# tudelft-iv/CCVPE

Measured on NVIDIA B200. Metric: VIGOR pairs/sec (CVM_VIGOR forward + pose decode, 320x640 panorama + 512x512 aerial), higher is better.
Workload: dtype bf16

## Files before the change

ccvpe_b200/csrc/encoder_ops.cu:

```cuda
#include <cstdlib>
#include <cstring>

#include "common.cuh"

namespace ccvpe {

constexpr float kSeFixedScale = 1048576.f;
__device__ __forceinline__ unsigned long long se_fixed(float v) {
  return (unsigned long long)__float2ll_rn(v * kSeFixedScale);
}

__global__ void __launch_bounds__(256)
bias_silu_nhwc_kernel(const __nv_bfloat16* __restrict__ x, const __nv_bfloat16* __restrict__ bias,
                      __nv_bfloat16* __restrict__ y, int64_t y_sb, int64_t y_sh, int64_t y_sw, int H, int W, int C,
                      int pix_per_block, long long* __restrict__ chan_sum) {
  extern __shared__ unsigned long long s_sum[];
  const int G = C >> 3;
  const int lanes = blockDim.x / G;
  const int cg = threadIdx.x % G, pl = threadIdx.x / G;
  const int b = blockIdx.y;
  const int HW = H * W;
  const int p_lo = blockIdx.x * pix_per_block;
  const int p_hi = min(HW, p_lo + pix_per_block);
  if (chan_sum) {
    for (int c = threadIdx.x; c < C; c += blockDim.x) s_sum[c] = 0ull;
    __syncthreads();
  }
  float bv[8] = {0.f, 0.f, 0.f, 0.f, 0.f, 0.f, 0.f, 0.f};
  if (bias && pl < lanes) {
    uint4 q = *reinterpret_cast<const uint4*>(bias + cg * 8);
    const __nv_bfloat162* h = reinterpret_cast<const __nv_bfloat162*>(&q);
#pragma unroll
    for (int j = 0; j < 4; ++j) {
      float2 f = __bfloat1622float2(h[j]);
      bv[2 * j] = f.x;
      bv[2 * j + 1] = f.y;
    }
  }
  float acc[8] = {0.f, 0.f, 0.f, 0.f, 0.f, 0.f, 0.f, 0.f};
  if (pl < lanes) {
    const __nv_bfloat16* xb = x + (int64_t)b * HW * C + cg * 8;
    __nv_bfloat16* yb = y + (int64_t)b * y_sb + cg * 8;
    constexpr int U = 4;
    for (int p0 = p_lo + pl; p0 < p_hi; p0 += lanes * U) {
      uint4 q[U];
#pragma unroll
      for (int u = 0; u < U; ++u) {
        const int p = p0 + u * lanes;
        if (p < p_hi) q[u] = __ldcs(reinterpret_cast<const uint4*>(xb + (int64_t)p * C));
      }
#pragma unroll
      for (int u = 0; u < U; ++u) {
        const int p = p0 + u * lanes;
        if (p >= p_hi) break;
        __nv_bfloat162* h = reinterpret_cast<__nv_bfloat162*>(&q[u]);
#pragma unroll
        for (int j = 0; j < 4; ++j) {
          float2 f = __bfloat1622float2(h[j]);
          float a0 = f.x + bv[2 * j], a1 = f.y + bv[2 * j + 1];
          a0 = __fdividef(a0, 1.f + __expf(-a0));
          a1 = __fdividef(a1, 1.f + __expf(-a1));
          h[j] = __floats2bfloat162_rn(a0, a1);
          if (chan_sum) {
            float2 r = __bfloat1622float2(h[j]);
            acc[2 * j] += r.x;
            acc[2 * j + 1] += r.y;
          }
        }
        const int hh = p / W, ww = p - hh * W;
        *reinterpret_cast<uint4*>(yb + hh * y_sh + ww * y_sw) = q[u];
      }
    }
  }
  if (chan_sum) {
    if (pl < lanes) {
#pragma unroll
      for (int j = 0; j < 8; ++j) atomicAdd(&s_sum[cg * 8 + j], se_fixed(acc[j]));
    }
    __syncthreads();
    for (int c = threadIdx.x; c < C; c += blockDim.x)
      atomicAdd(reinterpret_cast<unsigned long long*>(chan_sum) + (int64_t)b * C + c, s_sum[c]);
  }
}

}

extern "C" int ccvpe_bias_silu_nhwc(const void* x, const void* bias, void* y, int64_t y_sb, int64_t y_sh, int64_t y_sw,
                                    int B, int H, int W, int C, int64_t* chan_sum, void* stream) {
  using namespace ccvpe;
  CCVPE_REQUIRE(x && y, "ccvpe_bias_silu_nhwc: null pointer");
  CCVPE_REQUIRE(B > 0 && H > 0 && W > 0 && C > 0 && C % 8 == 0 && C <= 2048, "ccvpe_bias_silu_nhwc: bad shape B=%d H=%d W=%d C=%d",
                B, H, W, C);
  CCVPE_REQUIRE(aligned16(x) && aligned16(y) && aligned16(bias), "ccvpe_bias_silu_nhwc: pointers must be 16-byte aligned");
  CCVPE_REQUIRE(y_sw % 8 == 0 && y_sh % 8 == 0 && y_sb % 8 == 0, "ccvpe_bias_silu_nhwc: output strides must be multiples of 8");
  const int G = C / 8;
  CCVPE_REQUIRE(G <= 256, "ccvpe_bias_silu_nhwc: C too large");
  const int lanes = 256 / G;
  const int64_t HW = (int64_t)H * W;
  int blocks_x = (int)((8LL * sm_count() + B - 1) / B);
  int64_t ppb = (HW + blocks_x - 1) / blocks_x;
  ppb = (ppb + lanes - 1) / lanes * lanes;
  if (ppb < lanes) ppb = lanes;
  blocks_x = (int)((HW + ppb - 1) / ppb);
  bias_silu_nhwc_kernel<<<dim3(blocks_x, B), 256, chan_sum ? C * sizeof(unsigned long long) : 0, (cudaStream_t)stream>>>(
      (const __nv_bfloat16*)x, (const __nv_bfloat16*)bias, (__nv_bfloat16*)y, y_sb, y_sh, y_sw, H, W, C, (int)ppb, reinterpret_cast<long long*>(chan_sum));
  CCVPE_LAUNCH_CHECK("bias_silu_nhwc_kernel");
  return CCVPE_OK;
}

namespace ccvpe {

__device__ __forceinline__ float dw_tanh(float x) {
  float y;
  asm("tanh.approx.f32 %0, %1;" : "=f"(y) : "f"(x));
  return y;
}

template <int V> struct DwVec;
template <> struct DwVec<8> { using type = uint4; };
template <> struct DwVec<4> { using type = uint2; };
template <int V>
__device__ __forceinline__ void dw_widen(const typename DwVec<V>::type& q, uint64_t (&f)[V / 2]);
template <>
__device__ __forceinline__ void dw_widen<8>(const uint4& q, uint64_t (&f)[4]) {
  f[0] = bf16x2_to_f32x2(q.x);
  f[1] = bf16x2_to_f32x2(q.y);
  f[2] = bf16x2_to_f32x2(q.z);
  f[3] = bf16x2_to_f32x2(q.w);
}
template <>
__device__ __forceinline__ void dw_widen<4>(const uint2& q, uint64_t (&f)[2]) {
  f[0] = bf16x2_to_f32x2(q.x);
  f[1] = bf16x2_to_f32x2(q.y);
}

template <int K, int S, int V>
__global__ void __launch_bounds__(256, V == 8 ? 2 : 3)
dwconv_bias_silu_kernel(const __nv_bfloat16* __restrict__ x, int64_t x_sb, int64_t x_sh, int64_t x_sw,
                        const __nv_bfloat16* __restrict__ w, const __nv_bfloat16* __restrict__ bias,
                        __nv_bfloat16* __restrict__ y, int Ho, int Wo, int C, int CG, int strips_per_block,
                        long long* __restrict__ chan_sum) {
  using vec_t = typename DwVec<V>::type;
  constexpr int P = V / 2;
  constexpr int TW = 4;
  constexpr int IW = (TW - 1) * S + K;
  extern __shared__ __align__(16) float s_part[];
  const int CC = CG * V;
  float* s_w = s_part + (blockDim.x / CG) * CC;
  const int G = C / V;
  const int g0 = blockIdx.z * CG;
  const int gn = min(CG, G - g0);
  const int lanes = blockDim.x / CG;
  const int cl = threadIdx.x % CG, pl = threadIdx.x / CG;
  const int cg = g0 + cl;
  const bool active = pl < lanes && cl < gn;
  const int b = blockIdx.y;
  {
    const int q4 = gn * V / 4, n_items = K * K * q4;
#pragma unroll 1
    for (int i0 = threadIdx.x; i0 < n_items; i0 += 4 * blockDim.x) {
      uint2 v[4];
      int dst[4];
#pragma unroll
      for (int u = 0; u < 4; ++u) {
        const int i = i0 + u * blockDim.x;
        const int ii = i < n_items ? i : 0;
        const int tap = ii / q4, c4 = ii - tap * q4;
        v[u] = __ldg(reinterpret_cast<const uint2*>(w + (int64_t)tap * C + g0 * V) + c4);
        dst[u] = i < n_items ? tap * CC + c4 * 4 : -1;
      }
#pragma unroll
      for (int u = 0; u < 4; ++u)
        if (dst[u] >= 0)
          *reinterpret_cast<float4*>(s_w + dst[u]) =
              make_float4(0.5f * __uint_as_float(v[u].x << 16), 0.5f * __uint_as_float(v[u].x & 0xffff0000u),
                          0.5f * __uint_as_float(v[u].y << 16), 0.5f * __uint_as_float(v[u].y & 0xffff0000u));
    }
  }
  const int strips_row = (Wo + TW - 1) / TW;
  const int n_strips = Ho * strips_row;
  const int s_lo = blockIdx.x * strips_per_block;
  const int s_hi = min(n_strips, s_lo + strips_per_block);
  __syncthreads();
  float csum[V];
#pragma unroll
  for (int j = 0; j < V; ++j) csum[j] = 0.f;
  if (active) {
    uint64_t bv[P];
    dw_widen<V>(*reinterpret_cast<const vec_t*>(bias + cg * V), bv);
#pragma unroll
    for (int j = 0; j < P; ++j) {
      float lo, hi;
      unpack_f32x2(bv[j], lo, hi);
      bv[j] = pack_f32x2(0.5f * lo, 0.5f * hi);
    }
    const __nv_bfloat16* xb = x + (int64_t)b * x_sb + cg * V;
    __nv_bfloat16* yb = y + (int64_t)b * Ho * Wo * C + cg * V;
    const float* wt = s_w + cl * V;
    const int iw_max = (Wo - 1) * S + K - 1;
    const int sw = (int)x_sw;
    for (int sidx = s_lo + pl; sidx < s_hi; sidx += lanes) {
      const int ho = sidx / strips_row;
      const int wo0 = (sidx - ho * strips_row) * TW;
      uint64_t acc[TW][P];
#pragma unroll
      for (int t = 0; t < TW; ++t)
#pragma unroll
        for (int j = 0; j < P; ++j) acc[t][j] = bv[j];
      const int ix_max = iw_max - wo0 * S;
      const __nv_bfloat16* xrow = xb + (int64_t)(ho * S) * x_sh + (int64_t)(wo0 * S) * x_sw;
#pragma unroll 1
      for (int ky = 0; ky < K; ++ky, xrow += x_sh) {
        vec_t xin[IW];
#pragma unroll
        for (int ix = 0; ix < IW; ++ix)
          xin[ix] = __ldg(reinterpret_cast<const vec_t*>(xrow + min(ix, ix_max) * sw));
        uint64_t xf[IW][P];
#pragma unroll
        for (int kx = 0; kx < K; ++kx) {
          uint64_t wv[P];
// ... 177 lines not shown
            if (ky >= 0 && ky < K) {
              const uint2 wq = dwt_lds64(sw + (uint32_t)(ky * K + kx) * 128u);
              const uint64_t w0 = bf16x2_to_f32x2(wq.x), w1 = bf16x2_to_f32x2(wq.y);
#pragma unroll
              for (int t = 0; t < TW; ++t) {
                acc[r][t][0] = ffma2(xf[t + kx][0], w0, acc[r][t][0]);
                acc[r][t][1] = ffma2(xf[t + kx][1], w1, acc[r][t][1]);
              }
            }
          }
        }
      }
      const int ho0 = th_i * p.oth + ph * TH, wo0 = tw_i * p.otw + pw * TW;
#pragma unroll
      for (int r = 0; r < TH; ++r) {
        const int ho = ho0 + r;
        if (ho < p.Ho) {
          __nv_bfloat16* yrow = p.y + (((int64_t)b * p.Ho + ho) * p.Wo) * p.C + c0 + cg * 4;
#pragma unroll
          for (int t = 0; t < TW; ++t) {
            const int wo = wo0 + t;
            if (wo < p.Wo) {
              uint2 q;
              __nv_bfloat162* h = reinterpret_cast<__nv_bfloat162*>(&q);
#pragma unroll
              for (int j = 0; j < 2; ++j) {
                float a0, a1;
                unpack_f32x2(acc[r][t][j], a0, a1);
                a0 *= 0.5f;
                a1 *= 0.5f;
                a0 = fmaf(a0, dw_tanh(a0), a0);
                a1 = fmaf(a1, dw_tanh(a1), a1);
                h[j] = __floats2bfloat162_rn(a0, a1);
                const float2 rr = __bfloat1622float2(h[j]);
                csum[2 * j] += rr.x;
                csum[2 * j + 1] += rr.y;
              }
              *reinterpret_cast<uint2*>(yrow + (int64_t)wo * p.C) = q;
            }
          }
        }
      }
    }
    if (p.chan_sum) {
#pragma unroll
      for (int j = 0; j < 4; ++j) s_part[pt * DWT_CB + cg * 4 + j] = csum[j];
    }
    __syncthreads();
    if (p.chan_sum && tid < DWT_CB && c0 + tid < p.C) {
      float tot = 0.f;
#pragma unroll
      for (int l = 0; l < DWT_PT; ++l) tot += s_part[l * DWT_CB + tid];
      atomicAdd(reinterpret_cast<unsigned long long*>(p.chan_sum) + (int64_t)b * p.C + c0 + tid, se_fixed(tot));
    }
  }
}

static bool dwt_plan(int K, int Ho, int Wo, int C, int B, DwTileParams* p) {
  double best = 1e30;
  bool found = false;
  for (int ptw = 1; ptw <= DWT_PT; ++ptw) {
    const int pth = DWT_PT / ptw;
    const int otw = ptw * DWT_TW, oth = pth * DWT_TH;
    const int itw = otw + K - 1, ith = oth + K - 1;
    const int stage = (K * K + ith * itw) * 128;
    if (stage > DWT_STAGE_LIMIT) continue;
    const int tiles_w = (Wo + otw - 1) / otw, tiles_h = (Ho + oth - 1) / oth;
    const double cost = (double)tiles_w * tiles_h * (ith * itw + 2.0 * DWT_PT * DWT_TW * DWT_TH);
    if (cost < best) {
      best = cost;
      found = true;
      p->ptw = ptw; p->pth = pth; p->otw = otw; p->oth = oth; p->itw = itw; p->ith = ith;
      p->tiles_w = tiles_w; p->tiles_h = tiles_h; p->stage_bytes = stage;
    }
  }
  if (!found) return false;
  p->cblocks = (C + DWT_CB - 1) / DWT_CB;
  const int64_t total = (int64_t)p->tiles_w * p->tiles_h * p->cblocks * B;
  if (total > (1LL << 30)) return false;
  p->total_items = (int)total;
  return true;
}

__global__ void __launch_bounds__(512)
se_gate_scale_kernel(const long long* __restrict__ chan_sum, float inv_hw, const __nv_bfloat16* __restrict__ w_red,
                     const __nv_bfloat16* __restrict__ b_red, const __nv_bfloat16* __restrict__ w_se_t,
                     const __nv_bfloat16* __restrict__ b_se, const __nv_bfloat16* __restrict__ w_proj,
                     __nv_bfloat16* __restrict__ wg, int mid, int R, int cout, int rows_per_block) {
  extern __shared__ __align__(16) float s_se[];
  float* s_mean = s_se;
  float* s_h = s_se + mid;
  const int b = blockIdx.x, tid = threadIdx.x, lane = tid & 31, warp = tid >> 5;
  for (int m = tid; m < mid; m += blockDim.x) s_mean[m] = __ll2float_rn(chan_sum[(int64_t)b * mid + m]) * (inv_hw * (1.f / kSeFixedScale));
  __syncthreads();
  const int n_warps = blockDim.x >> 5;
  for (int r = warp; r < R; r += n_warps) {
    const __nv_bfloat16* wr = w_red + (int64_t)r * mid;
    float acc = 0.f;
    for (int m0 = lane * 8; m0 < mid; m0 += 256) {
      const uint4 q = __ldg(reinterpret_cast<const uint4*>(wr + m0));
      const __nv_bfloat162* hq = reinterpret_cast<const __nv_bfloat162*>(&q);
#pragma unroll
      for (int j = 0; j < 4; ++j) {
        const float2 f = __bfloat1622float2(hq[j]);
        acc = fmaf(f.x, s_mean[m0 + 2 * j], acc);
        acc = fmaf(f.y, s_mean[m0 + 2 * j + 1], acc);
      }
    }
#pragma unroll
    for (int o = 16; o > 0; o >>= 1) acc += __shfl_xor_sync(0xffffffffu, acc, o);
    if (lane == 0) {
      const float v = acc + __bfloat162float(b_red[r]);
      s_h[r] = __fdividef(v, 1.f + __expf(-v));
    }
  }
  __syncthreads();
  for (int m = tid; m < mid; m += blockDim.x) {
    float acc = __bfloat162float(b_se[m]);
#pragma unroll 8
    for (int r = 0; r < R; ++r) acc = fmaf(__bfloat162float(__ldg(w_se_t + (int64_t)r * mid + m)), s_h[r], acc);
    s_mean[m] = __fdividef(1.f, 1.f + __expf(-acc));
  }
  __syncthreads();
  const int c_lo = blockIdx.y * rows_per_block, c_hi = min(cout, c_lo + rows_per_block);
  const int vec_per_row = mid >> 3;
  const int total = (c_hi - c_lo) * vec_per_row;
  const uint4* src = reinterpret_cast<const uint4*>(w_proj + (int64_t)c_lo * mid);
  uint4* dst = reinterpret_cast<uint4*>(wg + ((int64_t)b * cout + c_lo) * mid);
  for (int i = tid; i < total; i += blockDim.x) {
    const int m0 = (i % vec_per_row) * 8;
    uint4 q = __ldg(src + i);
    __nv_bfloat162* hq = reinterpret_cast<__nv_bfloat162*>(&q);
#pragma unroll
    for (int j = 0; j < 4; ++j) {
      const float2 f = __bfloat1622float2(hq[j]);
      hq[j] = __floats2bfloat162_rn(f.x * s_mean[m0 + 2 * j], f.y * s_mean[m0 + 2 * j + 1]);
    }
    dst[i] = q;
  }
}

__global__ void __launch_bounds__(1024)
se_gate_kernel(const long long* __restrict__ chan_sum, float inv_hw, const __nv_bfloat16* __restrict__ w_red,
               const __nv_bfloat16* __restrict__ b_red, const __nv_bfloat16* __restrict__ w_se_t,
               const __nv_bfloat16* __restrict__ b_se, float* __restrict__ gate, int mid, int R) {
  extern __shared__ __align__(16) float s_se[];
  float* s_mean = s_se;
  float* s_h = s_se + mid;
  const int b = blockIdx.x, tid = threadIdx.x, lane = tid & 31, warp = tid >> 5;
  for (int m = tid; m < mid; m += blockDim.x) s_mean[m] = __ll2float_rn(chan_sum[(int64_t)b * mid + m]) * (inv_hw * (1.f / kSeFixedScale));
  __syncthreads();
  const int n_warps = blockDim.x >> 5;
  for (int r = warp; r < R; r += n_warps) {
    const __nv_bfloat16* wr = w_red + (int64_t)r * mid;
    float acc = 0.f;
    for (int m0 = lane * 8; m0 < mid; m0 += 256) {
      const uint4 q = __ldg(reinterpret_cast<const uint4*>(wr + m0));
      const __nv_bfloat162* hq = reinterpret_cast<const __nv_bfloat162*>(&q);
#pragma unroll
      for (int j = 0; j < 4; ++j) {
        const float2 f = __bfloat1622float2(hq[j]);
        acc = fmaf(f.x, s_mean[m0 + 2 * j], acc);
        acc = fmaf(f.y, s_mean[m0 + 2 * j + 1], acc);
      }
    }
#pragma unroll
// ... 115 lines not shown

extern "C" int ccvpe_stem_conv_silu_nhwc(const float* x, int B, int H, int W, const float* w, const float* bias, int CO,
                                         void* out, int in_pad_lo, int in_pad_hi, int out_pad_lo, int out_pad_hi,
                                         int circular, void* stream) {
  using namespace ccvpe;
  CCVPE_REQUIRE(x && w && bias && out, "ccvpe_stem_conv_silu_nhwc: null pointer");
  CCVPE_REQUIRE(B > 0 && H >= 3 && W >= 3 && B <= 65535, "ccvpe_stem_conv_silu_nhwc: bad shape B=%d H=%d W=%d", B, H, W);
  CCVPE_REQUIRE(CO == 32, "ccvpe_stem_conv_silu_nhwc: CO=%d unsupported (EfficientNet-B0 stem has 32 channels)", CO);
  CCVPE_REQUIRE(in_pad_lo >= 0 && in_pad_lo <= 2 && in_pad_hi >= 0 && in_pad_hi <= 2 && out_pad_lo >= 0 && out_pad_hi >= 0,
                "ccvpe_stem_conv_silu_nhwc: bad padding");
  CCVPE_REQUIRE(aligned16(out), "ccvpe_stem_conv_silu_nhwc: out must be 16-byte aligned");
  const int Ho = (H + in_pad_lo + in_pad_hi - 3) / 2 + 1, Wo = (W + in_pad_lo + in_pad_hi - 3) / 2 + 1;
  CCVPE_REQUIRE(!circular || (out_pad_lo <= Wo && out_pad_hi <= Wo), "ccvpe_stem_conv_silu_nhwc: wrap wider than the image");
  const int Hp = Ho + out_pad_lo + out_pad_hi, Wp = Wo + out_pad_lo + out_pad_hi;
  cudaStream_t st = (cudaStream_t)stream;
  StemTcParams tp;
  memset(&tp, 0, sizeof(tp));
  tp.x = x; tp.w = w; tp.bias = bias; tp.out = (__nv_bfloat16*)out;
  tp.B = B; tp.H = H; tp.W = W; tp.Ho = Ho; tp.Wo = Wo; tp.in_lo = in_pad_lo; tp.out_lo = out_pad_lo; tp.Hp = Hp; tp.Wp = Wp;
  return stem_tcgen05(tp, circular != 0, false, st);
}

extern "C" int ccvpe_stem_conv_silu_u8_nhwc(const uint8_t* x, int B, int H, int Wsrc, int crop_w, const int32_t* shift,
                                            const float* mean_host, const float* std_host, const float* w, const float* bias,
                                            int CO, void* out, int in_pad_lo, int in_pad_hi, int out_pad_lo, int out_pad_hi,
                                            int circular, void* stream) {
  using namespace ccvpe;
  CCVPE_REQUIRE(x && w && bias && out && mean_host && std_host, "ccvpe_stem_conv_silu_u8_nhwc: null pointer");
  const int W = crop_w;
  CCVPE_REQUIRE(B > 0 && H >= 3 && W >= 3 && W <= Wsrc && B <= 65535, "ccvpe_stem_conv_silu_u8_nhwc: bad shape B=%d H=%d W=%d Wsrc=%d",
                B, H, W, Wsrc);
  CCVPE_REQUIRE(CO == 32, "ccvpe_stem_conv_silu_u8_nhwc: CO=%d unsupported (EfficientNet-B0 stem has 32 channels)", CO);
  CCVPE_REQUIRE(in_pad_lo >= 0 && in_pad_lo <= 2 && in_pad_hi >= 0 && in_pad_hi <= 2 && out_pad_lo >= 0 && out_pad_hi >= 0,
                "ccvpe_stem_conv_silu_u8_nhwc: bad padding");
  CCVPE_REQUIRE(aligned16(out), "ccvpe_stem_conv_silu_u8_nhwc: out must be 16-byte aligned");
  const int Ho = (H + in_pad_lo + in_pad_hi - 3) / 2 + 1, Wo = (W + in_pad_lo + in_pad_hi - 3) / 2 + 1;
  CCVPE_REQUIRE(!circular || (out_pad_lo <= Wo && out_pad_hi <= Wo), "ccvpe_stem_conv_silu_u8_nhwc: wrap wider than the image");
  const int Hp = Ho + out_pad_lo + out_pad_hi, Wp = Wo + out_pad_lo + out_pad_hi;
  StemTcParams tp;
  memset(&tp, 0, sizeof(tp));
  tp.x8 = x; tp.shift = shift; tp.Wsrc = Wsrc;
  for (int c = 0; c < 3; ++c) {
    tp.sc[c] = 1.f / (255.f * std_host[c]);
    tp.sh[c] = -mean_host[c] / std_host[c];
  }
  tp.w = w; tp.bias = bias; tp.out = (__nv_bfloat16*)out;
  tp.B = B; tp.H = H; tp.W = W; tp.Ho = Ho; tp.Wo = Wo; tp.in_lo = in_pad_lo; tp.out_lo = out_pad_lo; tp.Hp = Hp; tp.Wp = Wp;
  return stem_tcgen05(tp, circular != 0, true, (cudaStream_t)stream);
}

extern "C" int ccvpe_pointwise_silu_nhwc(const void* x, int B, int H, int W, int K, int ldx, const void* w_nk,
                                         const float* bias, int N, void* out, int pad_lo, int pad_hi, void* stream) {
  using namespace ccvpe;
  CCVPE_REQUIRE(x && w_nk && out, "ccvpe_pointwise_silu_nhwc: null pointer");
  CCVPE_REQUIRE(B > 0 && H > 0 && W > 0 && (int64_t)B * H * W < (1LL << 31) - 256, "ccvpe_pointwise_silu_nhwc: bad shape");
  CCVPE_REQUIRE(K > 0 && K % 8 == 0 && N > 0 && N % 8 == 0 && ldx >= K && ldx % 8 == 0,
                "ccvpe_pointwise_silu_nhwc: K=%d N=%d ldx=%d must be positive multiples of 8", K, N, ldx);
  CCVPE_REQUIRE(pad_lo >= 0 && pad_hi >= 0, "ccvpe_pointwise_silu_nhwc: negative padding");
  CCVPE_REQUIRE(aligned16(x) && aligned16(w_nk) && aligned16(out), "ccvpe_pointwise_silu_nhwc: pointers must be 16-byte aligned");
  ccvpe_igemm_desc d;
  memset(&d, 0, sizeof(d));
  d.a0 = x; d.c0 = K; d.ld0 = ldx;
  d.B = B; d.Hin = d.Hout = H; d.Win = d.Wout = W;
  d.stride = 1; d.kh = d.kw = 1; d.pad = 0;
  d.N = N; d.dtype = CCVPE_BF16; d.w_nk = w_nk; d.bias = bias;
  d.relu = 2;
  d.out_mode = 0; d.out_dtype = CCVPE_BF16; d.ldo = N; d.out = out;
  d.backend = CCVPE_BACKEND_TCGEN05;
  const TcOutPad padded = {H + pad_lo + pad_hi, W + pad_lo + pad_hi, pad_lo};
  return igemm_tcgen05(d, (cudaStream_t)stream, (pad_lo || pad_hi) ? &padded : nullptr);
}

extern "C" int ccvpe_dwconv_bias_silu_nhwc(const void* x, int64_t x_sb, int64_t x_sh, int64_t x_sw, int Hp, int Wp,
                                           const void* w, const void* bias, void* y, int B, int C, int K, int S,
                                           int64_t* chan_sum, void* stream) {
  using namespace ccvpe;
  CCVPE_REQUIRE(x && w && bias && y, "ccvpe_dwconv_bias_silu_nhwc: null pointer");
  CCVPE_REQUIRE(B > 0 && C > 0 && C % 8 == 0 && C <= 2048, "ccvpe_dwconv_bias_silu_nhwc: bad shape B=%d C=%d", B, C);
  CCVPE_REQUIRE((K == 3 || K == 5) && (S == 1 || S == 2) && Hp >= K && Wp >= K, "ccvpe_dwconv_bias_silu_nhwc: K=%d S=%d Hp=%d Wp=%d unsupported", K, S, Hp, Wp);
  CCVPE_REQUIRE(aligned16(x) && aligned16(w) && aligned16(bias) && aligned16(y), "ccvpe_dwconv_bias_silu_nhwc: pointers must be 16-byte aligned");
  CCVPE_REQUIRE(x_sb % 8 == 0 && x_sh % 8 == 0 && x_sw % 8 == 0, "ccvpe_dwconv_bias_silu_nhwc: input strides must be multiples of 8");
  CCVPE_REQUIRE(x_sw > 0 && x_sw * 16 < (1LL << 31), "ccvpe_dwconv_bias_silu_nhwc: pixel stride out of range");
  const int Ho = (Hp - K) / S + 1, Wo = (Wp - K) / S + 1;
  static const int use_tiled = getenv("CCVPE_DW_TILED") ? atoi(getenv("CCVPE_DW_TILED")) : 1;
  if (S == 1 && (use_tiled == 2 || (use_tiled == 1 && (K == 5 || C >= 240)))) {
    DwTileParams tp;
    memset(&tp, 0, sizeof(tp));
    if (dwt_plan(K, Ho, Wo, C, B, &tp)) {
      tp.x = (const __nv_bfloat16*)x; tp.x_sb = x_sb; tp.x_sh = x_sh; tp.x_sw = x_sw; tp.Hp = Hp; tp.Wp = Wp;
      tp.w = (const __nv_bfloat16*)w; tp.bias = (const __nv_bfloat16*)bias; tp.y = (__nv_bfloat16*)y;
      tp.Ho = Ho; tp.Wo = Wo; tp.C = C;
      tp.chan_sum = reinterpret_cast<long long*>(chan_sum);
      const int smem = DWT_SCRATCH + 2 * tp.stage_bytes;
      static thread_local uint64_t tiled_attr = 0;
      if (first_use_on_device(tiled_attr)) {
        cudaFuncSetAttribute(dwconv_tile_kernel<3>, cudaFuncAttributeMaxDynamicSharedMemorySize, DWT_SCRATCH + 2 * DWT_STAGE_LIMIT);
        cudaFuncSetAttribute(dwconv_tile_kernel<5>, cudaFuncAttributeMaxDynamicSharedMemorySize, DWT_SCRATCH + 2 * DWT_STAGE_LIMIT);
      }
      const int max_grid = 2 * sm_count();
      const int grid = tp.total_items < max_grid ? tp.total_items : max_grid;
      if (K == 3) dwconv_tile_kernel<3><<<grid, DWT_THREADS, smem, (cudaStream_t)stream>>>(tp);
      else dwconv_tile_kernel<5><<<grid, DWT_THREADS, smem, (cudaStream_t)stream>>>(tp);
      CCVPE_LAUNCH_CHECK("dwconv_tile_kernel");
      return CCVPE_OK;
    }
  }
  static const int force_v = getenv("CCVPE_DW_V") ? atoi(getenv("CCVPE_DW_V")) : 0;
  const int V = force_v ? force_v : 8;
  const int G = C / V;
  int CG = G;
  if (C > 256) {
    CG = 128 / V;
    for (int c = 128 / V; c >= 64 / V; --c)
      if (G % c == 0) {
        CG = c;
        break;
      }
  }
  const int chunks = (G + CG - 1) / CG;
  const int lanes = 256 / CG;
  const int64_t n_strips = (int64_t)Ho * ((Wo + 3) / 4);
  int blocks_x = (int)((8LL * sm_count() + (int64_t)B * chunks - 1) / ((int64_t)B * chunks));
  int64_t spb = (n_strips + blocks_x - 1) / blocks_x;
  spb = (spb + lanes - 1) / lanes * lanes;
  if (spb < lanes) spb = lanes;
  blocks_x = (int)((n_strips + spb - 1) / spb);
  CCVPE_REQUIRE(chunks <= 65535 && B <= 65535, "ccvpe_dwconv_bias_silu_nhwc: grid too large");
  const dim3 grid(blocks_x, B, chunks);
  const size_t sm = (size_t)CG * V * sizeof(float) * (lanes + K * K);
  CCVPE_REQUIRE(sm <= 96 * 1024, "ccvpe_dwconv_bias_silu_nhwc: K*K*C too large for shared memory");
  static thread_local uint64_t attr_set = 0;
  if (first_use_on_device(attr_set)) {
#define CCVPE_DW_ATTR(KK, SS, VV) \
  cudaFuncSetAttribute(dwconv_bias_silu_kernel<KK, SS, VV>, cudaFuncAttributeMaxDynamicSharedMemorySize, 96 * 1024)
    CCVPE_DW_ATTR(3, 1, 8); CCVPE_DW_ATTR(3, 2, 8); CCVPE_DW_ATTR(5, 1, 8); CCVPE_DW_ATTR(5, 2, 8);
    CCVPE_DW_ATTR(3, 1, 4); CCVPE_DW_ATTR(3, 2, 4); CCVPE_DW_ATTR(5, 1, 4); CCVPE_DW_ATTR(5, 2, 4);
#undef CCVPE_DW_ATTR
  }
  cudaStream_t st = (cudaStream_t)stream;
#define CCVPE_DW(KK, SS, VV)                                                                                          \
  dwconv_bias_silu_kernel<KK, SS, VV><<<grid, 256, sm, st>>>((const __nv_bfloat16*)x, x_sb, x_sh, x_sw,               \
                                                             (const __nv_bfloat16*)w, (const __nv_bfloat16*)bias,     \
                                                             (__nv_bfloat16*)y, Ho, Wo, C, CG, (int)spb, reinterpret_cast<long long*>(chan_sum))
  if (V == 8) {
    if (K == 3 && S == 1) CCVPE_DW(3, 1, 8);
    else if (K == 3 && S == 2) CCVPE_DW(3, 2, 8);
    else if (K == 5 && S == 1) CCVPE_DW(5, 1, 8);
    else CCVPE_DW(5, 2, 8);
  } else {
    if (K == 3 && S == 1) CCVPE_DW(3, 1, 4);
    else if (K == 3 && S == 2) CCVPE_DW(3, 2, 4);
    else if (K == 5 && S == 1) CCVPE_DW(5, 1, 4);
    else CCVPE_DW(5, 2, 4);
  }
#undef CCVPE_DW
  CCVPE_LAUNCH_CHECK("dwconv_bias_silu_kernel");
  return CCVPE_OK;
}
```

ccvpe_b200/csrc/tcgen05_common.cuh:

```cuda
#pragma once

#include <cuda.h>

#include <cstdlib>
#include <mutex>

#include "common.cuh"

namespace ccvpe {

constexpr int TC_BM = 128;
constexpr int TC_MAX_N = 256;
constexpr int TC_EPI_WARPS = 8;
constexpr int TC_EPI_THREADS = 32 * TC_EPI_WARPS;

__device__ __forceinline__ uint32_t smem_u32(const void* p) { return (uint32_t)__cvta_generic_to_shared(p); }

__device__ __forceinline__ bool elect_one() {
  uint32_t pred;
  asm volatile(
      "{\n\t.reg .pred P;\n\t"
      "elect.sync _|P, 0xffffffff;\n\t"
      "selp.u32 %0, 1, 0, P;\n\t}"
      : "=r"(pred));
// ... 299 lines not shown
      *reinterpret_cast<uint4*>(my + g8 * 16) = pk;
    };
    if (c0 + 32 <= ncols) {
      group(0);
      group(1);
      group(2);
      group(3);
    } else {
#pragma unroll
      for (int g8 = 0; g8 < 4; ++g8)
        if (c0 + g8 * 8 < ncols) group(g8);
    }
    __syncwarp();
    const bool unit_ok = fc < ((min(32, ncols - c0)) >> 3);
    const int goff = unit_ok ? (s_off[(c0 >> 3) + fc] >> 3) : 0;
#pragma unroll
    for (int pass = 0; pass < 4; ++pass) {
      const int32_t rb = s_rowbase[pass * 8 + fr];
      const uint4 val = *reinterpret_cast<const uint4*>(src + pass * 8 * EPI_CHUNK_PITCH);
      if (unit_ok && rb >= 0) out16[(uint32_t)(rb + goff)] = val;
    }
    __syncwarp();
  }
}

inline bool tc_epilogue_supported(const ccvpe_igemm_desc& d) {
  if (d.out_dtype != CCVPE_BF16) return true;
  if (d.out_mode == 2) return false;
  const int cout = d.out_mode == 1 ? d.N / 4 : d.N;
  const int64_t out_elems = (int64_t)(d.out_mode == 1 ? 4 : 1) * d.B * d.Hout * d.Wout * d.ldo;
  return (cout % 8 == 0) && (d.ldo % 8 == 0) && ((reinterpret_cast<uintptr_t>(d.out) & 15) == 0) &&
         (d.out_mode != 1 || d.N % 4 == 0) && out_elems < (1LL << 33);
}

inline int epi_variant(const EpiParams& e) {
  if (e.relu == 2) return 6;
  if (e.out_mode == 1) return e.row_r1 ? 5 : 4;
  if (e.out_mode == 2) return 3;
  if (e.out_f32) return 2;
  return e.row_r1 ? 1 : 0;
}
#define CCVPE_EPI_SWITCH(variant, X) \
  switch (variant) {                 \
    case 0: X(0, false, false); break; \
    case 1: X(0, true, false); break;  \
    case 2: X(0, false, true); break;  \
    case 3: X(2, false, true); break;  \
    case 4: X(1, false, false); break; \
    default: X(1, true, false); break; \
  }

typedef CUresult (*EncodeTiledFn)(CUtensorMap*, CUtensorMapDataType, cuuint32_t, void*, const cuuint64_t*,
                                  const cuuint64_t*, const cuuint32_t*, const cuuint32_t*, CUtensorMapInterleave,
                                  CUtensorMapSwizzle, CUtensorMapL2promotion, CUtensorMapFloatOOBfill);

inline EncodeTiledFn encode_fn() {
  static EncodeTiledFn fn = nullptr;
  static std::once_flag once;
  std::call_once(once, [] {
    void* sym = nullptr;
    cudaDriverEntryPointQueryResult qres;
    if (cudaGetDriverEntryPointByVersion("cuTensorMapEncodeTiled", &sym, 12000, cudaEnableDefault, &qres) == cudaSuccess &&
        qres == cudaDriverEntryPointSuccess)
      fn = reinterpret_cast<EncodeTiledFn>(sym);
  });
  return fn;
}

inline int encode_map(CUtensorMap* tm, const void* base, int rank, const uint64_t* dims, const uint64_t* strides_bytes,
                      const uint32_t* box, int kw) {
  EncodeTiledFn fn = encode_fn();
  if (!fn) return fail(CCVPE_ERR_CUDA, "cuTensorMapEncodeTiled entry point not available");
  cuuint64_t gdim[5];
  cuuint64_t gstr[4];
  cuuint32_t bx[5], es[5];
  for (int i = 0; i < rank; ++i) {
    gdim[i] = dims[i];
    bx[i] = box[i];
    es[i] = 1;
  }
  for (int i = 0; i + 1 < rank; ++i) gstr[i] = strides_bytes[i];
  CUresult r = fn(tm, CU_TENSOR_MAP_DATA_TYPE_BFLOAT16, (cuuint32_t)rank, const_cast<void*>(base), gdim, gstr, bx, es,
                  CU_TENSOR_MAP_INTERLEAVE_NONE,
                  kw == 64 ? CU_TENSOR_MAP_SWIZZLE_128B : (kw == 32 ? CU_TENSOR_MAP_SWIZZLE_64B : CU_TENSOR_MAP_SWIZZLE_32B),
                  CU_TENSOR_MAP_L2_PROMOTION_L2_256B,
                  CU_TENSOR_MAP_FLOAT_OOB_FILL_NONE);
  if (r != CUDA_SUCCESS)
    return fail(CCVPE_ERR_CUDA, "cuTensorMapEncodeTiled failed (%d) rank=%d dims=[%llu,%llu,%llu,..] box=[%u,%u,%u,..]",
                (int)r, rank, (unsigned long long)dims[0], (unsigned long long)dims[1],
                (unsigned long long)(rank > 2 ? dims[2] : 0), box[0], box[1], rank > 2 ? box[2] : 0);
  return CCVPE_OK;
}


inline int tc_block_width(int c) {
  static const bool old_rule = getenv("CCVPE_KW_OLD") != nullptr;
  return c <= 16 ? 16 : (c < (old_rule ? 64 : 33) ? 32 : 64);
}
inline int tc_block_width_match(int c) {
  static const bool old_rule = getenv("CCVPE_MATCH_KW_OLD") != nullptr;
  return c <= 16 ? 16 : (c < (old_rule ? 64 : 33) ? 32 : 64);
}

inline void fill_epi(EpiParams& e, const ccvpe_igemm_desc& d) {
  e.N = d.N;
  e.HWo = d.Hout * d.Wout;
  e.Wout = d.Wout;
  e.Hout = d.Hout;
  e.bias = d.bias;
  e.row_scale = d.row_scale;
  e.row_r1 = d.row_r1;
  e.r1_w = d.r1_w;
  e.relu = d.relu;
  e.out_mode = d.out_mode;
  e.out_f32 = (d.out_dtype == CCVPE_F32);
  e.ldo = d.ldo;
  e.out = d.out;
}

}
```

Before: 5795.

## Add TMA-fed persistent depthwise conv kernel with per-channel-block tiling

Adds a new stride-1 depthwise conv kernel that loads input halo tiles with TMA into a double-buffered shared-memory ring guarded by mbarriers. Each CTA is persistent over a channel block and walks spatial tiles. Threads compute 2x8 output micro-tiles with packed f32x2 FMAs and fuse bias, SiLU and the SE channel-sum reduction. Routing sends all K=3 stride-1 convs and K=5 convs with C<=240 to this path and strips the unused V=4 and K=3 tiled variants. The gain depends on TMA overlap beating the older register-strip kernels. The risk is weaker occupancy or bank conflicts, since the tensor map uses no swizzle.

```diff
diff --git a/ccvpe_b200/csrc/encoder_ops.cu b/ccvpe_b200/csrc/encoder_ops.cu
--- a/ccvpe_b200/csrc/encoder_ops.cu
+++ b/ccvpe_b200/csrc/encoder_ops.cu
@@ -2,6 +2,7 @@
 #include <cstring>
 
 #include "common.cuh"
+#include "tcgen05_common.cuh"
 
 namespace ccvpe {
 
@@ -118,7 +119,6 @@
 
 template <int V> struct DwVec;
 template <> struct DwVec<8> { using type = uint4; };
-template <> struct DwVec<4> { using type = uint2; };
 template <int V>
 __device__ __forceinline__ void dw_widen(const typename DwVec<V>::type& q, uint64_t (&f)[V / 2]);
 template <>
@@ -128,14 +128,9 @@
   f[2] = bf16x2_to_f32x2(q.z);
   f[3] = bf16x2_to_f32x2(q.w);
 }
-template <>
-__device__ __forceinline__ void dw_widen<4>(const uint2& q, uint64_t (&f)[2]) {
-  f[0] = bf16x2_to_f32x2(q.x);
-  f[1] = bf16x2_to_f32x2(q.y);
-}
 
 template <int K, int S, int V>
-__global__ void __launch_bounds__(256, V == 8 ? 2 : 3)
+__global__ void __launch_bounds__(256, 2)
 dwconv_bias_silu_kernel(const __nv_bfloat16* __restrict__ x, int64_t x_sb, int64_t x_sh, int64_t x_sw,
                         const __nv_bfloat16* __restrict__ w, const __nv_bfloat16* __restrict__ bias,
                         __nv_bfloat16* __restrict__ y, int Ho, int Wo, int C, int CG, int strips_per_block,
@@ -479,6 +474,247 @@
   return true;
 }
 
+constexpr int DW_THREADS = 256;
+constexpr int DW_STAGES = 2;
+constexpr int DW_STAGE_LIMIT = 48 * 1024;
+
+constexpr int DW_TH = 2, DW_TW = 8;
+
+struct DwParams {
+  CUtensorMap tmap;
+  const __nv_bfloat16* w;
+  const __nv_bfloat16* bias;
+  __nv_bfloat16* y;
+  long long* chan_sum;
+  int Ho, Wo, C;
+  int cb, lanes, ptw, pth, otw, oth, itw, ith;
+  int tiles_w, tiles_h, items, ctas_per_cb;
+  int box_bytes, stage_bytes, stage_off;
+};
+
+__device__ __forceinline__ float4 dw_lds128(uint32_t addr) {
+  float4 v;
+  asm volatile("ld.shared.v4.f32 {%0, %1, %2, %3}, [%4];" : "=f"(v.x), "=f"(v.y), "=f"(v.z), "=f"(v.w) : "r"(addr));
+  return v;
+}
+
+template <int K, int S, int CB>
+__global__ void __launch_bounds__(DW_THREADS, 2) dwconv_tma_kernel(const __grid_constant__ DwParams p) {
+  constexpr int TH = DW_TH, TW = DW_TW;
+  constexpr int IH = (TH - 1) * S + K, IW = (TW - 1) * S + K;
+  extern __shared__ __align__(128) uint8_t dw_smem[];
+  constexpr int cb = CB, LANES = CB / 4, PT = DW_THREADS / LANES;
+  float* s_w = reinterpret_cast<float*>(dw_smem);
+  float* s_bias = s_w + K * K * cb;
+  float* s_part = s_bias + cb;
+  uint64_t* s_bar = reinterpret_cast<uint64_t*>(s_part + 2 * PT * cb);
+  const uint32_t stage0 = smem_u32(dw_smem) + (uint32_t)p.stage_off;
+  const int tid = threadIdx.x;
+  const int cg = tid % LANES, pt = tid / LANES;
+  const int pw = pt % p.ptw, ph = pt / p.ptw;
+  const int npt = p.ptw * p.pth;
+  const bool active = pt < npt;
+  const int cblk = blockIdx.x / p.ctas_per_cb, first = blockIdx.x - cblk * p.ctas_per_cb;
+  const int c0 = cblk * cb;
+
+  if (tid == 0) {
+    for (int s = 0; s < DW_STAGES; ++s) mbar_init(smem_u32(&s_bar[s]), 1);
+    asm volatile("fence.mbarrier_init.release.cluster;" ::: "memory");
+    prefetch_tmap(&p.tmap);
+  }
+  auto issue = [&](int item, int stage) {
+    const int tw_i = item % p.tiles_w, rest = item / p.tiles_w;
+    const int th_i = rest % p.tiles_h, b = rest / p.tiles_h;
+    const uint32_t bar = smem_u32(&s_bar[stage]);
+    mbar_arrive_expect_tx(bar, (uint32_t)p.box_bytes);
+    tma_load_4d(stage0 + (uint32_t)(stage * p.stage_bytes), &p.tmap, bar, c0, tw_i * p.otw * S, th_i * p.oth * S, b);
+  };
+  {
+    const int q4 = cb >> 2, n = K * K * q4;
+    for (int i = tid; i < n; i += blockDim.x) {
+      const int tap = i / q4, c4 = i - tap * q4;
+      const uint2 v = __ldg(reinterpret_cast<const uint2*>(p.w + (int64_t)tap * p.C + c0) + c4);
+      *reinterpret_cast<float4*>(s_w + tap * cb + c4 * 4) =
+          make_float4(__uint_as_float(v.x << 16), __uint_as_float(v.x & 0xffff0000u), __uint_as_float(v.y << 16),
+                      __uint_as_float(v.y & 0xffff0000u));
+    }
+    for (int c = tid; c < cb; c += blockDim.x) s_bias[c] = __bfloat162float(p.bias[c0 + c]);
+  }
+  __syncthreads();
+  if (tid == 0) {
+    for (int s = 0; s < DW_STAGES; ++s)
+      if (first + s * p.ctas_per_cb < p.items) issue(first + s * p.ctas_per_cb, s);
+  }
+  constexpr uint32_t pix = CB * 2;
+  const uint32_t row_pitch = (uint32_t)p.itw * pix;
+  const uint32_t s_wt = smem_u32(s_w + cg * 4);
+  const uint32_t x_off = (uint32_t)(ph * TH * S) * row_pitch + (uint32_t)(pw * TW * S) * pix + (uint32_t)cg * 8u;
+
+  int it = 0;
+  for (int item = first; item < p.items; item += p.ctas_per_cb, ++it) {
+    const int stage = it % DW_STAGES;
+    float csum[4] = {0.f, 0.f, 0.f, 0.f};
+    mbar_wait(smem_u32(&s_bar[stage]), (uint32_t)((it / DW_STAGES) & 1));
+    if (active) {
+      const uint32_t sx = stage0 + (uint32_t)(stage * p.stage_bytes) + x_off;
+      uint64_t acc[TH][TW][2];
+      {
+        const float4 bq = dw_lds128(s_wt + (uint32_t)(K * K * cb) * 4u);
+#pragma unroll
+        for (int r = 0; r < TH; ++r)
+#pragma unroll
+          for (int t = 0; t < TW; ++t) {
+            acc[r][t][0] = pack_f32x2(bq.x, bq.y);
+            acc[r][t][1] = pack_f32x2(bq.z, bq.w);
+          }
+      }
+#pragma unroll (K == 3 ? IH : 1)
+      for (int ir = 0; ir < IH; ++ir) {
+        uint64_t xf[IW][2];
+#pragma unroll
+        for (int kx = 0; kx < K; ++kx) {
+#pragma unroll
+          for (int t = 0; t < TW; ++t)
+            if (kx < S || t == TW - 1) {
+              const int ix = t * S + kx;
+              const uint2 v = dwt_lds64(sx + (uint32_t)ir * row_pitch + (uint32_t)ix * pix);
+              xf[ix][0] = bf16x2_to_f32x2(v.x);
+              xf[ix][1] = bf16x2_to_f32x2(v.y);
+            }
+#pragma unroll
+          for (int r = 0; r < TH; ++r) {
+            const int ky = ir - r * S;
+            if (ky >= 0 && ky < K) {
+              const float4 wq = dw_lds128(s_wt + (uint32_t)((ky * K + kx) * cb) * 4u);
+              const uint64_t w0 = pack_f32x2(wq.x, wq.y), w1 = pack_f32x2(wq.z, wq.w);
+#pragma unroll
+              for (int t = 0; t < TW; ++t) {
+                acc[r][t][0] = ffma2(xf[t * S + kx][0], w0, acc[r][t][0]);
+                acc[r][t][1] = ffma2(xf[t * S + kx][1], w1, acc[r][t][1]);
+              }
+            }
+          }
+        }
+      }
+      const int tw_i = item % p.tiles_w, rest = item / p.tiles_w;
+      const int th_i = rest % p.tiles_h, b = rest / p.tiles_h;
+      const int ho0 = th_i * p.oth + ph * TH, wo0 = tw_i * p.otw + pw * TW;
+#pragma unroll
+      for (int r = 0; r < TH; ++r) {
+        const int ho = ho0 + r;
+        if (ho < p.Ho) {
+          __nv_bfloat16* yrow = p.y + (((int64_t)b * p.Ho + ho) * p.Wo) * p.C + c0 + cg * 4;
+#pragma unroll
+          for (int t = 0; t < TW; ++t) {
+            const int wo = wo0 + t;
+            if (wo < p.Wo) {
+              uint2 q;
+              __nv_bfloat162* h = reinterpret_cast<__nv_bfloat162*>(&q);
+#pragma unroll
+              for (int j = 0; j < 2; ++j) {
+                float a0, a1;
+                unpack_f32x2(acc[r][t][j], a0, a1);
+                a0 *= 0.5f;
+                a1 *= 0.5f;
+                a0 = fmaf(a0, dw_tanh(a0), a0);
+                a1 = fmaf(a1, dw_tanh(a1), a1);
+                h[j] = __floats2bfloat162_rn(a0, a1);
+                const float2 rr = __bfloat1622float2(h[j]);
+                csum[2 * j] += rr.x;
+                csum[2 * j + 1] += rr.y;
+              }
+              *reinterpret_cast<uint2*>(yrow + (int64_t)wo * p.C) = q;
+            }
+          }
+        }
+      }
+    }
+    float* part = s_part + (it & 1) * PT * cb;
+    if (p.chan_sum && active) *reinterpret_cast<float4*>(part + pt * cb + cg * 4) = make_float4(csum[0], csum[1], csum[2], csum[3]);
+    __syncthreads();
+    if (tid == 0 && item + DW_STAGES * p.ctas_per_cb < p.items) issue(item + DW_STAGES * p.ctas_per_cb, stage);
+    if (p.chan_sum && tid < cb) {
+      float tot = 0.f;
+      for (int l = 0; l < npt; ++l) tot += part[l * cb + tid];
+      const int b = item / (p.tiles_w * p.tiles_h);
+      atomicAdd(reinterpret_cast<unsigned long long*>(p.chan_sum) + (int64_t)b * p.C + c0 + tid, se_fixed(tot));
+    }
+  }
+}
+
+static int dw_block(int C) { return C % 64 == 0 ? 64 : (C % 48 == 0 ? 48 : (C % 32 == 0 ? 32 : 8)); }
+
+static int dw_plan(int K, int S, int Ho, int Wo, int C, int B, DwParams* p) {
+  const int TH = DW_TH, TW = DW_TW;
+  const int cb = dw_block(C);
+  const int lanes = cb / 4, max_pt = DW_THREADS / lanes;
+  double best = 1e30;
+  for (int ptw = 1; ptw <= max_pt; ++ptw)
+    for (int pth = 1; pth <= max_pt / ptw; ++pth) {
+      const int otw = ptw * TW, oth = pth * TH;
+      const int itw = (otw - 1) * S + K, ith = (oth - 1) * S + K;
+      const int stage = (itw * ith * cb * 2 + 127) / 128 * 128;
+      if (itw > 256 || ith > 256 || stage > DW_STAGE_LIMIT) continue;
+      const double tiles = (double)((Wo + otw - 1) / otw) * ((Ho + oth - 1) / oth);
+      const double cost = tiles * ((double)itw * ith + 2.0 * max_pt * TW * TH);
+      if (cost < best) {
+        best = cost;
+        p->ptw = ptw; p->pth = pth; p->otw = otw; p->oth = oth; p->itw = itw; p->ith = ith;
+        p->box_bytes = itw * ith * cb * 2;
+        p->stage_bytes = stage;
+      }
+    }
+  if (best == 1e30) return fail(CCVPE_ERR_UNSUPPORTED, "dwconv: no tile plan for K=%d S=%d C=%d", K, S, C);
+  p->cb = cb; p->lanes = lanes;
+  p->tiles_w = (Wo + p->otw - 1) / p->otw;
+  p->tiles_h = (Ho + p->oth - 1) / p->oth;
+  const int64_t items = (int64_t)B * p->tiles_w * p->tiles_h;
+  if (items > (1LL << 30)) return fail(CCVPE_ERR_UNSUPPORTED, "dwconv: too many tiles (B=%d %dx%d)", B, Ho, Wo);
+  p->items = (int)items;
+  const int cblocks = C / cb;
+  int per = 2 * sm_count() / cblocks;
+  if (per < 1) per = 1;
+  if (per > p->items) per = p->items;
+  p->ctas_per_cb = per;
+  const int fixed = (K * K * cb + cb + 2 * DW_THREADS * 4) * 4 + DW_STAGES * 8;
+  p->stage_off = (fixed + 127) / 128 * 128;
+  return CCVPE_OK;
+}
+
+static int dwconv_tma(const void* x, int64_t x_sb, int64_t x_sh, int64_t x_sw, int Hp, int Wp, const void* w,
+                      const void* bias, void* y, int B, int C, int K, int Ho, int Wo, int64_t* chan_sum, cudaStream_t stream) {
+  constexpr int S = 1;
+  DwParams p;
+  memset(&p, 0, sizeof(p));
+  int rc = dw_plan(K, S, Ho, Wo, C, B, &p);
+  if (rc != CCVPE_OK) return rc;
+  {
+    const uint64_t dims[4] = {(uint64_t)C, (uint64_t)Wp, (uint64_t)Hp, (uint64_t)B};
+    const uint64_t str[3] = {(uint64_t)x_sw * 2, (uint64_t)x_sh * 2, (uint64_t)x_sb * 2};
+    const uint32_t box[4] = {(uint32_t)p.cb, (uint32_t)p.itw, (uint32_t)p.ith, 1};
+    if ((rc = encode_map(&p.tmap, x, 4, dims, str, box, 0)) != CCVPE_OK) return rc;
+  }
+  p.w = (const __nv_bfloat16*)w; p.bias = (const __nv_bfloat16*)bias; p.y = (__nv_bfloat16*)y;
+  p.chan_sum = reinterpret_cast<long long*>(chan_sum);
+  p.Ho = Ho; p.Wo = Wo; p.C = C;
+  const int smem = p.stage_off + DW_STAGES * p.stage_bytes;
+  using DwKernel = void (*)(DwParams);
+#define CCVPE_DW_K(KK) {dwconv_tma_kernel<KK, S, 64>, dwconv_tma_kernel<KK, S, 48>, dwconv_tma_kernel<KK, S, 32>, dwconv_tma_kernel<KK, S, 8>}
+  static const DwKernel kernels[2][4] = {CCVPE_DW_K(3), CCVPE_DW_K(5)};
+#undef CCVPE_DW_K
+  const DwKernel fn = kernels[K == 5][p.cb == 64 ? 0 : (p.cb == 48 ? 1 : (p.cb == 32 ? 2 : 3))];
+  static thread_local uint64_t attr = 0;
+  if (first_use_on_device(attr)) {
+    const int max_smem = 64 * 1024 + DW_STAGES * DW_STAGE_LIMIT;
+    for (auto& row : kernels)
+      for (DwKernel k : row) cudaFuncSetAttribute(k, cudaFuncAttributeMaxDynamicSharedMemorySize, max_smem);
+  }
+  const int grid = (C / p.cb) * p.ctas_per_cb;
+  fn<<<grid, DW_THREADS, smem, stream>>>(p);
+  CCVPE_LAUNCH_CHECK("dwconv_tma_kernel");
+  return CCVPE_OK;
+}
+
 __global__ void __launch_bounds__(512)
 se_gate_scale_kernel(const long long* __restrict__ chan_sum, float inv_hw, const __nv_bfloat16* __restrict__ w_red,
                      const __nv_bfloat16* __restrict__ b_red, const __nv_bfloat16* __restrict__ w_se_t,
@@ -760,8 +996,9 @@
   CCVPE_REQUIRE(x_sb % 8 == 0 && x_sh % 8 == 0 && x_sw % 8 == 0, "ccvpe_dwconv_bias_silu_nhwc: input strides must be multiples of 8");
   CCVPE_REQUIRE(x_sw > 0 && x_sw * 16 < (1LL << 31), "ccvpe_dwconv_bias_silu_nhwc: pixel stride out of range");
   const int Ho = (Hp - K) / S + 1, Wo = (Wp - K) / S + 1;
-  static const int use_tiled = getenv("CCVPE_DW_TILED") ? atoi(getenv("CCVPE_DW_TILED")) : 1;
-  if (S == 1 && (use_tiled == 2 || (use_tiled == 1 && (K == 5 || C >= 240)))) {
+  if (S == 1 && (K == 3 || C <= 240))
+    return dwconv_tma(x, x_sb, x_sh, x_sw, Hp, Wp, w, bias, y, B, C, K, Ho, Wo, chan_sum, (cudaStream_t)stream);
+  if (S == 1) {
     DwTileParams tp;
     memset(&tp, 0, sizeof(tp));
     if (dwt_plan(K, Ho, Wo, C, B, &tp)) {
@@ -771,20 +1008,16 @@
       tp.chan_sum = reinterpret_cast<long long*>(chan_sum);
       const int smem = DWT_SCRATCH + 2 * tp.stage_bytes;
       static thread_local uint64_t tiled_attr = 0;
-      if (first_use_on_device(tiled_attr)) {
-        cudaFuncSetAttribute(dwconv_tile_kernel<3>, cudaFuncAttributeMaxDynamicSharedMemorySize, DWT_SCRATCH + 2 * DWT_STAGE_LIMIT);
+      if (first_use_on_device(tiled_attr))
         cudaFuncSetAttribute(dwconv_tile_kernel<5>, cudaFuncAttributeMaxDynamicSharedMemorySize, DWT_SCRATCH + 2 * DWT_STAGE_LIMIT);
-      }
       const int max_grid = 2 * sm_count();
       const int grid = tp.total_items < max_grid ? tp.total_items : max_grid;
-      if (K == 3) dwconv_tile_kernel<3><<<grid, DWT_THREADS, smem, (cudaStream_t)stream>>>(tp);
-      else dwconv_tile_kernel<5><<<grid, DWT_THREADS, smem, (cudaStream_t)stream>>>(tp);
+      dwconv_tile_kernel<5><<<grid, DWT_THREADS, smem, (cudaStream_t)stream>>>(tp);
       CCVPE_LAUNCH_CHECK("dwconv_tile_kernel");
       return CCVPE_OK;
     }
   }
-  static const int force_v = getenv("CCVPE_DW_V") ? atoi(getenv("CCVPE_DW_V")) : 0;
-  const int V = force_v ? force_v : 8;
+  constexpr int V = 8;
   const int G = C / V;
   int CG = G;
   if (C > 256) {
@@ -811,8 +1044,7 @@
   if (first_use_on_device(attr_set)) {
 #define CCVPE_DW_ATTR(KK, SS, VV) \
   cudaFuncSetAttribute(dwconv_bias_silu_kernel<KK, SS, VV>, cudaFuncAttributeMaxDynamicSharedMemorySize, 96 * 1024)
-    CCVPE_DW_ATTR(3, 1, 8); CCVPE_DW_ATTR(3, 2, 8); CCVPE_DW_ATTR(5, 1, 8); CCVPE_DW_ATTR(5, 2, 8);
-    CCVPE_DW_ATTR(3, 1, 4); CCVPE_DW_ATTR(3, 2, 4); CCVPE_DW_ATTR(5, 1, 4); CCVPE_DW_ATTR(5, 2, 4);
+    CCVPE_DW_ATTR(3, 2, 8); CCVPE_DW_ATTR(5, 1, 8); CCVPE_DW_ATTR(5, 2, 8);
 #undef CCVPE_DW_ATTR
   }
   cudaStream_t st = (cudaStream_t)stream;
@@ -820,17 +1052,9 @@
   dwconv_bias_silu_kernel<KK, SS, VV><<<grid, 256, sm, st>>>((const __nv_bfloat16*)x, x_sb, x_sh, x_sw,               \
                                                              (const __nv_bfloat16*)w, (const __nv_bfloat16*)bias,     \
                                                              (__nv_bfloat16*)y, Ho, Wo, C, CG, (int)spb, reinterpret_cast<long long*>(chan_sum))
-  if (V == 8) {
-    if (K == 3 && S == 1) CCVPE_DW(3, 1, 8);
-    else if (K == 3 && S == 2) CCVPE_DW(3, 2, 8);
-    else if (K == 5 && S == 1) CCVPE_DW(5, 1, 8);
-    else CCVPE_DW(5, 2, 8);
-  } else {
-    if (K == 3 && S == 1) CCVPE_DW(3, 1, 4);
-    else if (K == 3 && S == 2) CCVPE_DW(3, 2, 4);
-    else if (K == 5 && S == 1) CCVPE_DW(5, 1, 4);
-    else CCVPE_DW(5, 2, 4);
-  }
+  if (K == 3) CCVPE_DW(3, 2, 8);
+  else if (S == 1) CCVPE_DW(5, 1, 8);
+  else CCVPE_DW(5, 2, 8);
 #undef CCVPE_DW
   CCVPE_LAUNCH_CHECK("dwconv_bias_silu_kernel");
   return CCVPE_OK;
diff --git a/ccvpe_b200/csrc/tcgen05_common.cuh b/ccvpe_b200/csrc/tcgen05_common.cuh
--- a/ccvpe_b200/csrc/tcgen05_common.cuh
+++ b/ccvpe_b200/csrc/tcgen05_common.cuh
@@ -405,7 +405,7 @@
   for (int i = 0; i + 1 < rank; ++i) gstr[i] = strides_bytes[i];
   CUresult r = fn(tm, CU_TENSOR_MAP_DATA_TYPE_BFLOAT16, (cuuint32_t)rank, const_cast<void*>(base), gdim, gstr, bx, es,
                   CU_TENSOR_MAP_INTERLEAVE_NONE,
-                  kw == 64 ? CU_TENSOR_MAP_SWIZZLE_128B : (kw == 32 ? CU_TENSOR_MAP_SWIZZLE_64B : CU_TENSOR_MAP_SWIZZLE_32B),
+                  kw == 64 ? CU_TENSOR_MAP_SWIZZLE_128B : (kw == 32 ? CU_TENSOR_MAP_SWIZZLE_64B : (kw == 0 ? CU_TENSOR_MAP_SWIZZLE_NONE : CU_TENSOR_MAP_SWIZZLE_32B)),
                   CU_TENSOR_MAP_L2_PROMOTION_L2_256B,
                   CU_TENSOR_MAP_FLOAT_OOB_FILL_NONE);
   if (r != CUDA_SUCCESS)
```

Result: no change. 5845 (median of 6 runs) (+0.9%).
